# OzAmram/CaloDiffusion

Measured on AMD Instinct MI355X. Metric: sampled showers/sec (Dataset-2, 400-step DDIM), higher is better.
Workload: dtype f32 (convs: fp32 operands as 2-term fp16 splits on the fp16 MFMA pipe, fp32 accumulate; attention/norms fp32)

## Files before the change

### calodiffusion_amd/build.py

```python
from __future__ import annotations

import os
import subprocess
import sys
from concurrent.futures import ThreadPoolExecutor

HERE = os.path.dirname(os.path.abspath(__file__))
CSRC = os.path.join(HERE, "csrc")
LIBDIR = os.path.join(HERE, "lib")
TAG = os.environ.get("CD_BUILD_TAG", "")
LIB = os.path.join(LIBDIR, f"libcalodiff_hip{'_' + TAG if TAG else ''}.so")
SOURCES = ["kernels_conv.hip", "kernels_conv_zs.hip", "kernels_attn.hip", "kernels_conv_small.hip", "kernels_deep.hip", "kernels_wgrad16.hip", "kernels_norm_attn.hip", "kernels_misc.hip", "kernels_mlp.hip", "kernels_mlp_train.hip", "kernels_bwd.hip", "profiler.hip", "plan.hip",
           "forward.hip", "sampler.hip", "train.hip", "bns.hip", "ops.hip", "misc_abi.hip"]
HIPCC = os.environ.get("HIPCC", "/opt/rocm/bin/hipcc")
FLAGS = ["--offload-arch=gfx950", "-O3", "-std=c++17", "-fPIC", "-fno-gpu-rdc", "-Wall", "-Wno-unused-function", "-Wno-unused-value"]
FLAGS += os.environ.get("CD_EXTRA_HIPCC_FLAGS", "").split()
FILE_FLAGS = {"kernels_conv_zs.hip": ["-mllvm", "-amdgpu-mfma-vgpr-form"]}


def _file_digest(paths, extra: str = "") -> str:
    import hashlib
    h = hashlib.sha256(extra.encode())
    for f in paths:
        h.update(os.path.basename(f).encode())
        h.update(open(f, "rb").read())
    return h.hexdigest()


def _read(path: str):
    try:
        return open(path).read().strip()
    except OSError:
        return None


def build_all(force: bool = False, verbose: bool = True) -> str:
    os.makedirs(LIBDIR, exist_ok=True)
    objdir = os.path.join(LIBDIR, "obj" + ("_" + TAG if TAG else ""))
    os.makedirs(objdir, exist_ok=True)
    inc = os.path.join(os.path.dirname(HERE), "include")
    headers = sorted(os.path.join(CSRC, f) for f in os.listdir(CSRC) if f.endswith((".h", ".inc")))
    headers += sorted(os.path.join(inc, f) for f in os.listdir(inc) if f.endswith(".h"))
    jobs = []
    objs = []
    for src in SOURCES:
        sp = os.path.join(CSRC, src)
        op = os.path.join(objdir, src.replace(".hip", ".o"))
        objs.append(op)
        flags = [*FLAGS, *FILE_FLAGS.get(os.path.basename(sp), [])]
        key = _file_digest([sp] + headers, " ".join(flags))
        if force or not os.path.exists(op) or _read(op + ".hash") != key:
            jobs.append(([HIPCC, *flags, "-c", sp, "-o", op], op, key))

    def run(cmd):
        if verbose:
            print(" ".join(cmd), flush=True)
        r = subprocess.run(cmd, capture_output=True, text=True)
        if r.returncode != 0:
            raise RuntimeError(f"hipcc failed:\n{r.stdout}\n{r.stderr}")
        if verbose and r.stderr.strip():
            print(r.stderr, file=sys.stderr)

    def compile_one(job):
        cmd, op, key = job
        if os.path.exists(op + ".hash"):
            os.remove(op + ".hash")
        run(cmd)
        with open(op + ".hash", "w") as fh:
            fh.write(key + "\n")

    with ThreadPoolExecutor(max_workers=4) as ex:
        list(ex.map(compile_one, jobs))
    want = source_hash()
    if force or jobs or not os.path.exists(LIB) or _read(LIB + ".srchash") != want:
        if os.path.exists(LIB + ".srchash"):
            os.remove(LIB + ".srchash")
        run([HIPCC, "--offload-arch=gfx950", "-shared", "-fPIC", "-o", LIB, *objs])
        with open(LIB + ".srchash", "w") as fh:
            fh.write(want + "\n")
    return LIB


def source_hash() -> str:
    import hashlib
    h = hashlib.sha256((" ".join(FLAGS) + repr(sorted(FILE_FLAGS.items()))).encode())
    inc = os.path.join(os.path.dirname(HERE), "include")
    files = [os.path.join(CSRC, f) for f in sorted(os.listdir(CSRC))] + [os.path.join(inc, f) for f in sorted(os.listdir(inc))]
    for f in files:
        if f.endswith((".hip", ".h", ".inc")):
            h.update(os.path.basename(f).encode())
            h.update(open(f, "rb").read())
    return h.hexdigest()


if __name__ == "__main__":
    print(build_all(force="--force" in sys.argv))
```

### calodiffusion_amd/csrc/cd_common.h

```cpp
#pragma once
#include <hip/hip_runtime.h>
#include <stdint.h>
#include <stddef.h>
#include <string>

typedef float f32x4 __attribute__((ext_vector_type(4)));
typedef float f32x16 __attribute__((ext_vector_type(16)));

struct CdSamplerOp;

namespace cd {

void set_error(const std::string& msg);
struct Fail {
  int code;
  std::string msg;
};
#define CD_HIP(expr)                                                                                  \
  do {                                                                                                \
    hipError_t _e = (expr);                                                                           \
    if (_e != hipSuccess)                                                                             \
      throw cd::Fail{-2, std::string(#expr) + ": " + hipGetErrorString(_e)};                          \
  } while (0)
#define CD_REQUIRE(cond, msg)                                                                         \
  do {                                                                                                \
    if (!(cond)) throw cd::Fail{-1, std::string(msg)};                                                \
  } while (0)

namespace prof {
bool enabled();
void begin();
int end(char* buf, int cap);
struct Scope {
  Scope(const char* category, hipStream_t s, double flops, double bytes);
  ~Scope();
  int idx;
  hipStream_t stream;
};
}

enum ConvPrecision { PREC_F16X2 = 0, PREC_BF16X3 = 1, PREC_F32 = 2 };
int conv_precision();
void set_conv_precision(int p);
void set_conv_precision_override(int p);

struct Dims3 {
  int d, h, w;
  __host__ __device__ int64_t vox() const { return (int64_t)d * h * w; }
};

inline size_t packed_weight_floats(int cin, int cout, int taps) {
  return (size_t)(cin / 32) * taps * ((cout + 31) / 32) * 2048;
}

struct ConvGeom {
  Dims3 in, out;
  int kd, kh, kw;
  int sz, sh, sw;
};

__device__ __forceinline__ float cd_fast_silu(float t) {
  return t * __builtin_amdgcn_rcpf(1.f + __builtin_amdgcn_exp2f(t * -1.4426950408889634f));
}

struct GnDefer {
  const float* part = nullptr;
  int units = 0;
  const float* gamma = nullptr;
  const float* beta = nullptr;
  const float* add = nullptr;
  int add_ld = 0;
  int C = 0, groups = 0;
  int64_t vox = 0;
  float* coef_out = nullptr;
  float* stat_out = nullptr;
};

struct ConvFusion {
  const float* coef = nullptr;
  int act = 0;
  float* ch_part = nullptr;
  int* units = nullptr;
  const void* wpk_bf16x3 = nullptr;
  int* status = nullptr;
  GnDefer defer;
  float* coef_buf = nullptr;
  const unsigned* in_absmax = nullptr;
  const float* add_src = nullptr;
  int* add_done = nullptr;
  struct GnOut {
    const float* gamma = nullptr;
    const float* beta = nullptr;
    int groups = 0;
    const float* res0 = nullptr;
    const float* res1 = nullptr;
    int res_c0 = 0;
    float* part_out = nullptr;
    int* done = nullptr;
  } gn_out;
};
struct AbsmaxWords {
  unsigned* next = nullptr;
  unsigned* end = nullptr;
  unsigned* take() {
    CD_REQUIRE(next && next < end, "internal: out of max-|x| words");
    return next++;
  }
};
const unsigned* launch_absmax_bits(const float* x, size_t n, AbsmaxWords* words, hipStream_t s);
__host__ __device__ inline void pow2_scale_for(unsigned mb, float* scale, float* inv) {
  const int e = (int)((mb >> 23) & 0xff) - 127;
  int sexp = mb == 0u ? 0 : 10 - e;
  sexp = sexp < -100 ? -100 : (sexp > 100 ? 100 : sexp);
  union { unsigned u; float f; } a, b;
  a.u = (unsigned)(127 + sexp) << 23;
  b.u = (unsigned)(127 - sexp) << 23;
  *scale = a.f;
  *inv = b.f;
}
inline size_t packed_bf16x3_bytes(int cin, int cout, int taps) {
  return (size_t)(cin / 16) * taps * ((cout + 31) / 32) * 3 * 64 * 16;
}
inline size_t packed_f16x2_bytes(int cin, int cout, int taps) {
  return (size_t)(cin / 16) * taps * ((cout + 31) / 32) * 2 * 64 * 16;
}
inline size_t packed_split16_bytes(int cin, int cout, int taps) {
  return packed_bf16x3_bytes(cin, cout, taps) + packed_f16x2_bytes(cin, cout, taps);
}
void launch_pack_weights_bf16x3(const float* w_torch, void* wpk, int cout, int cin, int taps, hipStream_t s,
                                bool transposed = false, bool flip = false);
void launch_pack_weights_f16x2(const float* w_torch, void* wpk, int cout, int cin, int taps, hipStream_t s,
                               bool transposed = false, bool flip = false);
inline void launch_pack_weights_split16(const float* w_torch, void* wpk, int cout, int cin, int taps, hipStream_t s,
                                        bool transposed = false, bool flip = false) {
  launch_pack_weights_bf16x3(w_torch, wpk, cout, cin, taps, s, transposed, flip);
  launch_pack_weights_f16x2(w_torch, (char*)wpk + packed_bf16x3_bytes(cin, cout, taps), cout, cin, taps, s, transposed, flip);
}

void launch_pack_weights(const float* w_torch, float* wpk, int cout, int cin, int taps, bool transposed, hipStream_t s,
                         bool flip = false);
void launch_pack_init_weights(const float* w_torch, float* wpk, int cout, int cin, hipStream_t s);
struct PackJob {
  const float* src;
  float* raw;
  float* pk;
  void* bf3;
  void* f16;
  int cout, cin, taps;
  int kind;
  int tr, flip;
  unsigned long long numel, n_pk, n_bf3, n_f16;
};
void launch_pack_jobs(const PackJob* d_jobs, int njobs, hipStream_t s);
void launch_pack_jobs_f16x2(const PackJob* d_jobs, int njobs, hipStream_t s);

void launch_conv_mfma(const float* in0, int c0, const float* in1, int c1, const float* wpk, const float* bias, float* out,
                      int batch, int cout, const ConvGeom& g, hipStream_t s, const ConvFusion& fu = ConvFusion());
bool try_launch_conv_zslide(const float* in0, int c0, const float* in1, int c1, const void* wpk_f16x2, const float* bias, float* out,
                            int batch, int cout, const ConvGeom& g, hipStream_t s, const ConvFusion& fu);
bool try_launch_conv_small(const float* in0, int c0, const float* in1, int c1, const void* wpk_f16x2, const float* bias, float* out,
                           int batch, int cout, const ConvGeom& g, hipStream_t s, const ConvFusion& fu);
void launch_conv_transpose_mfma(const float* in, int cin, const float* wpk, const float* bias, float* out, int batch,
                                int cout, Dims3 din, Dims3 dout, int kz, int sz, hipStream_t s,
                                const void* wpk_f16x2 = nullptr, int* status = nullptr, const unsigned* in_absmax = nullptr);

enum A_Prologue { A_NONE = 0, A_AFFINE = 1, A_SOFTMAX32 = 2, A_EXPNORM = 3 };
struct PointwiseArgs {
  const float* in0 = nullptr;
  int ld0 = 0, off0 = 0, c0 = 0;
  const float* in1 = nullptr;
  int ld1 = 0, c1 = 0;
  const float* wpk = nullptr;
  int64_t w_batch_stride = 0;
  const float* bias = nullptr;
  const float* residual = nullptr;
  float* out = nullptr;
  int batch = 0, cout = 0;
  int64_t vox = 0;
  int prologue = A_NONE;
  const float* coef = nullptr;
  int out_ld = 0, out_off = 0;
  float* ch_part = nullptr;
  const float* gn_res = nullptr;
  GnDefer gn_defer;
  const void* wpk16 = nullptr;
  int* status = nullptr;
};
inline int pointwise_units(int64_t vox) { return (int)((vox + 127) / 128); }
void launch_pointwise(const PointwiseArgs& a, hipStream_t s);

struct InitConvArgs {
  const float* x = nullptr;
  int cx = 0;
  int cin = 0;
  const float* scale_b = nullptr;
  int scale_stride = 1;
  const float* sigma_b = nullptr;
  float sigma_data = 1.f;
  const float* r_w = nullptr;
  const float* z_d = nullptr;
  const float* phi_h = nullptr;
  int use_rz = 0, use_phi = 0;
  const float* wpk = nullptr;
  const float* bias = nullptr;
  float* out = nullptr;
  int batch = 0, cout = 0;
  Dims3 dims{};
  float* coord_table = nullptr;
  bool table_ready = false;
  int* status = nullptr;
};
void launch_init_conv(const InitConvArgs& a, hipStream_t s);
void launch_init_coord_table(const InitConvArgs& a, hipStream_t s);

int gn_nsplit_for(int64_t vox, int batch);
void launch_ch_stats(const float* x, float* part, int batch, int channels, int64_t vox, int nsplit, hipStream_t s);
void launch_gn_finalize(const float* part, int units, const float* gamma, const float* beta, const float* add_bc, int add_ld,
                        float* coef, int batch, int channels, int groups, int64_t vox, hipStream_t s,
                        float* stat_out = nullptr );

size_t wgrad_partial_floats(int64_t out_vox, int batch, bool per_sample, int A, int Bc, int T);
struct WgradReduceJob {
  const float* partial;
  float* dw;
  int A, Bc, T, nslots, flags , b_total, b_off;
  unsigned first_block;
};
struct WgradReduceQueue {
  static constexpr int kMax = 80;
  WgradReduceJob job[kMax];
  int n = 0;
  unsigned blocks = 0;
};
void wgrad_queue_flush(WgradReduceQueue* q, hipStream_t s);
struct WgradAux {
  WgradReduceQueue* queue = nullptr;
  AbsmaxWords* words = nullptr;
  const unsigned* gmax = nullptr;
  const unsigned* xmax = nullptr;
};
void launch_wgrad(const float* g, int A, Dims3 dg, const float* x, int Bc, int xld, int xoff, Dims3 dx, int kd, int kh, int kw,
                  int sz, int sxy, int batch, bool per_sample, float* partial, float* dw, bool accumulate, bool transposed_out,
                  hipStream_t s, int b_total = 0, int b_off = 0,
                  const float* xcoef = nullptr, const WgradAux& aux = WgradAux());
bool wgrad_x_norm_supported(Dims3 dg, Dims3 dx, int kd, int kh, int kw, int sz, int sxy);
bool wgrad_f16x2_eligible(Dims3 d);
bool try_launch_wgrad_f16x2(const float* g, int A, const float* x, int Bc, int xld, int xoff, Dims3 d, int batch, float* partial,
                            const WgradAux& aux, int* nblk_out, hipStream_t s, const float* xcoef = nullptr);
bool try_launch_wgrad_strided_f16x2(const float* g, int A, Dims3 dg, const float* x, int Bc, int xld, int xoff, Dims3 dx, int kd, int sz,
                                    int batch, float* partial, int max_slots, const WgradAux& aux, int* nblk_out, hipStream_t s);
void launch_strided_dgrad_naive(const float* dy, const float* w, float* dx, int batch, int cin, int cout, Dims3 din, Dims3 dout,
                                int kd, int sz, hipStream_t s);
void launch_softmax32(const float* qkv, float* qs, int64_t rows, hipStream_t s);
void launch_softmax32_bwd(const float* qs, const float* dqs, float* dqkv, int64_t rows, hipStream_t s);
void launch_ksoftmax_bwd(const float* qkv, const float* dks, const float* kstat, const float* ctx, const float* dctx, float dscale,
                         float* dqkv, int batch, int64_t vox, hipStream_t s);
void launch_pack_sample32(const float* m, float* wpk, int batch, bool transpose, float scale, hipStream_t s);
void launch_pack_sample32_pair(const float* m, float* wpk_plain, float* wpk_tr, int batch, float scale, hipStream_t s);
int head_bwd_blocks(int batch, int64_t vox);
void launch_head_loss_bwd(const float* x0, const float* data, const float* noise, const float* scal, const float* h, const float* wh,
                          float* dh, float* part, float* dwh, float* dbh, int batch, int64_t vox, hipStream_t s, int loss_type = 0,
                          int objective = 0);
void launch_head_vjp(const float* gy, const float* scal, const float* h, const float* wh, float* dh, float* part, float* dwh, float* dbh,
                     int batch, int64_t vox, int objective, hipStream_t s);
void launch_init_dgrad(const float* g, const float* w_raw, int cin, int c0, const float* gy, const float* scal, int objective, float* dx,
                       int batch, Dims3 dims, hipStream_t s);
struct LinearWgradJob {
  const float* delta;
  const float* in;
  float* dw;
  float* db;
  int nout, nin, delta_ld, in_ld;
};
void launch_linear_wgrad(const LinearWgradJob* jobs_dev, int njobs, int max_elems, int batch, hipStream_t s);
void launch_fold_phi(const float* src, float* dst, int batch, Dims3 d, int C, hipStream_t s);
void launch_add_slices(const float* a, int lda, int aoff, const float* b, int ldb, int boff, float* out, int channels,
                       int64_t rows, hipStream_t s);
void launch_bias_grad(const float* part, int units, int batch, int channels, float* db, bool accumulate, hipStream_t s);
size_t gn_backward_scratch_floats(int batch, int channels, int64_t vox);
struct GnParamJob {
  const float* sums_bc;
  float *dgamma, *dbeta, *dbias, *dsumdy;
  int batch, channels;
};
struct GnParamJobs {
  static constexpr int kMax = 64;
  GnParamJob job[kMax];
  int n = 0;
};
struct GnParamQueue {
  GnParamJobs jobs;
  float* sums = nullptr;
  float* sums_end = nullptr;
  float* next_sums = nullptr;
  bool discard = false;
};
void launch_gn_param_jobs(const GnParamJobs& jobs, hipStream_t s);
void launch_gn_backward(const float* dy, const float* h, const float* coef, const float* stat, const float* gamma, float* dh,
                        float* dgamma, float* dbeta, float* dadd, int dadd_ld, int batch, int channels, int64_t vox, int groups,
                        int silu, float* scratch, bool accumulate_params, hipStream_t s,
                        float* dbias = nullptr, float* dsumdy = nullptr,
                        GnParamQueue* queue = nullptr,
                        unsigned* dh_absmax = nullptr);
int gn_apply_blocks_per_sample(int batch, int channels, int64_t vox);
void launch_gn_apply(const float* x, float* y, const float* coef, int batch, int channels, int64_t vox, int silu,
                     const float* residual, const float* residual1, int res_c0, float* part_out, hipStream_t s,
                     const GnDefer* defer = nullptr);

int attn_nsplit_for(int64_t vox, int batch);
size_t attn_partial_floats(int batch, int nsplit);
void launch_attn_context(const float* qkv, float* partials, int batch, int64_t vox, int nsplit, hipStream_t s);
void launch_attn_combine(const float* partials, int nsplit, const float* w_out , int cout, float* wpk_b,
// ... 272 lines not shown
```

### calodiffusion_amd/csrc/kernels_conv.hip

```cpp
#include "cd_common.h"
#include "split16.h"
#include "gn_defer.h"
#include <cstdio>
#include <cstdlib>
#include <cstring>
#include <algorithm>
#include <map>
#include <string>
#include <vector>

namespace cd {

static int g_conv_precision = -1;
static thread_local int tl_conv_precision_override = -1;
void set_conv_precision_override(int p) { tl_conv_precision_override = p; }
int conv_precision() {
  if (tl_conv_precision_override >= 0) return tl_conv_precision_override;
  if (g_conv_precision < 0) {
    const char* e = getenv("CD_CONV_PRECISION");
    g_conv_precision = !e ? PREC_F16X2 : (!strcmp(e, "f32") ? PREC_F32 : (!strcmp(e, "bf16x3") ? PREC_BF16X3 : PREC_F16X2));
  }
  return g_conv_precision;
}
void set_conv_precision(int p) { g_conv_precision = p; }
// ... 1476 lines not shown
  const bool bf16x3 = prec != 0;
  if (getenv("CD_NO_FLAT")) return false;
  int geo = -1;
  if (g.kd == 3 && g.kh == 3 && g.kw == 3 && g.sz == 1 && g.sh == 1 && g.sw == 1) geo = 0;
  else if (g.kd == 3 && g.kh == 4 && g.kw == 4 && g.sh == 2 && g.sw == 2 && (g.sz == 1 || g.sz == 2)) geo = g.sz == 2 ? 1 : 2;
  else if (g.kd == 4 && g.kh == 4 && g.kw == 4 && g.sh == 2 && g.sw == 2 && g.sz == 2) geo = 3;
  if (geo < 0 || (geo != 0 && !bf16x3)) return false;
  const Dims3 d = g.in;
  const int CTtot = cout / 32;
  const int CTmax = CTtot <= 3 ? CTtot : 2;
  if (CTtot % CTmax) return false;
  const int HW = d.h * d.w, HWo = g.out.h * g.out.w;
  const size_t vox_bytes = prec == 3 ? 96 : (prec == 2 ? 80 : 64);
  auto planes = [&](int NT) { return ((32 * NT - 1) / HWo + 1) * g.sz + g.kd; };
  auto launch = [&](int NT, int VT, int CT) -> bool {
    if (VT < 0) {
      const int NLW = -VT;
      ConvFlatArgs a;
      a.in0 = in0; a.in1 = in1; a.c0 = c0; a.c1 = c1; a.wpk = (const float*)wpk; a.bias = bias; a.out = out;
      a.D = d.d; a.H = d.h; a.W = d.w; a.Do = g.out.d; a.Ho = g.out.h; a.Wo = g.out.w;
      a.R = 32 * NT; a.P = planes(NT); a.cout = cout; a.CTtot = CTtot; a.dbg = 0;
      a.coef = fu.coef; a.act = fu.act; a.ch_part = fu.ch_part;
      const size_t lds = 2 * ((size_t)a.P * HW + 1) * 96 + (size_t)NT * CT * 64 * 4;
      const int ups = (int)((g.out.vox() + a.R - 1) / a.R);
      const int total = ups * batch;
      const int nblk = total < 256 ? total : 256;
      dim3 grid((unsigned)nblk, 1, (unsigned)(CTtot / CT));
      if (fu.units) *fu.units = ups;
      const int threads = (NT + NLW) * 64;
      switch (CT) {
        case 1: launch_ws_inst<1>(a, grid, threads, lds, NLW, ups, total, s, geo); break;
        case 2: launch_ws_inst<2>(a, grid, threads, lds, NLW, ups, total, s, geo); break;
        case 3: launch_ws_inst<3>(a, grid, threads, lds, NLW, ups, total, s, geo); break;
        default: return false;
      }
      return true;
    }
    ConvFlatArgs a;
    a.in0 = in0; a.in1 = in1; a.c0 = c0; a.c1 = c1; a.wpk = (const float*)wpk; a.bias = bias; a.out = out;
    a.D = d.d; a.H = d.h; a.W = d.w; a.Do = g.out.d; a.Ho = g.out.h; a.Wo = g.out.w;
    a.R = 32 * NT; a.P = planes(NT); a.cout = cout; a.CTtot = CTtot;
    a.dbg = getenv("CD_FLAT_DBG") ? atoi(getenv("CD_FLAT_DBG")) : 0;
    a.coef = fu.coef; a.act = fu.act; a.ch_part = fu.ch_part; a.status = fu.status; a.in_absmax = fu.in_absmax;
    a.add_src = prec >= 2 && !bias ? fu.add_src : nullptr;
    size_t lds = ((size_t)a.P * HW + 1) * vox_bytes;
    const size_t red = (size_t)(NT / VT) * CT * 32 * 2 * 4;
    if (lds < red) lds = red;
    if (fu.defer.part) {
      lds = (lds + 15) & ~(size_t)15;
      a.defer = fu.defer;
      a.coef_lds_off = (int)lds;
      lds += (size_t)fu.defer.C * 16 + gn_defer_scratch_bytes(fu.defer.C);
      if (lds > 160 * 1024) return false;
    }
    dim3 grid((unsigned)((g.out.vox() + a.R - 1) / a.R), (unsigned)batch, (unsigned)(CTtot / CT));
    if (fu.units) *fu.units = (int)grid.x;
    const int threads = (NT / VT) * 64;
#define CD_FLAT_CASE(V, C)                                                   \
  if (VT == V && CT == C) {                                                  \
    if (prec == 3) launch_flat3_inst<V, C, 3>(a, grid, threads, lds, s, geo); \
    else if (prec == 2) {                                                    \
      if constexpr (V * C <= 4) launch_flat3_inst<V, C, 2>(a, grid, threads, lds, s, geo); \
      else return false;                                                     \
    } else launch_flat_inst<V, C>(a, grid, threads, lds, s);                 \
    if (a.add_src && fu.add_done) *fu.add_done = 1;                          \
    return true;                                                             \
  }
    CD_FLAT_CASE(1, 1) CD_FLAT_CASE(2, 1) CD_FLAT_CASE(3, 1) CD_FLAT_CASE(4, 1)
    CD_FLAT_CASE(1, 2) CD_FLAT_CASE(2, 2) CD_FLAT_CASE(3, 2) CD_FLAT_CASE(4, 2)
    CD_FLAT_CASE(1, 3) CD_FLAT_CASE(2, 3)
#undef CD_FLAT_CASE
    return false;
  };
  if (const char* ov = getenv("CD_FLAT_TILE")) {
    int nt, vt;
    if (sscanf(ov, "%d,%d", &nt, &vt) == 2 && nt % vt == 0 && nt / vt <= 8 && vt * CTmax <= 8 &&
        ((size_t)planes(nt) * HW + 1) * vox_bytes <= 160 * 1024 && (prec != 2 || vt * CTmax <= 4))
      return launch(nt, vt, CTmax);
  }
  static const int kCand[][2] = {{8, 2}, {4, 1}, {8, 1}, {12, 3}, {16, 2}, {16, 4}, {4, 2}, {6, 2}, {6, 3}, {2, 1},
                                 {3, 1}, {1, 1}, {2, 2}, {12, 2}, {8, 4}, {6, 1}, {3, 3}};
  struct Cand { int nt, vt, ct; };
  std::vector<Cand> cand;
  const bool small = g.out.vox() * batch <= 64 * 1024;
  for (int pass = 0; pass < (small && CTmax > 1 ? 2 : 1); ++pass) {
    const int CT = pass == 0 ? CTmax : 1;
    for (auto& c : kCand) {
      const int NT = c[0], VT = c[1];
      if (VT * CT > 8 || (CT == 3 && VT > 2)) continue;
      if (prec == 2 && VT * CT > 4) continue;
      static const bool no_extra_waves = getenv("CD_FLAT_NO_EXTRA_WAVES") != nullptr;
      const bool extra_ok = !no_extra_waves && g.out.vox() <= 128 && VT == 1 && NT <= 8;
      if ((int64_t)32 * (NT - 1) >= g.out.vox() && !extra_ok) continue;
      if (((size_t)planes(NT) * HW + 1) * vox_bytes > 150 * 1024) continue;
      if (pass == 1 && NT > 4) continue;
      cand.push_back({NT, VT, CT});
    }
  }
  if (prec == 3 && !getenv("CD_NO_WS")) {
    static const int kWs[][2] = {{8, 4}, {8, 2}, {4, 2}, {4, 4}, {8, 3}, {6, 2}, {2, 2}, {3, 1}, {1, 1}, {2, 1}};
    for (auto& c : kWs) {
      const int NMW = c[0], NLW = c[1];
      if ((int64_t)32 * (NMW - 1) >= g.out.vox()) continue;
      const size_t lds = 2 * ((size_t)planes(NMW) * HW + 1) * 96 + (size_t)NMW * CTmax * 64 * 4;
      if (lds > 160 * 1024 - 256) continue;
      cand.push_back({NMW, -NLW, CTmax});
    }
  }
  if (cand.empty()) return false;
  char key[192];
  std::snprintf(key, sizeof key, "flat%s g%d %dx%dx%d c%d+%d->%d b%d", prec == 3 ? "_bf16x3" : (prec == 2 ? "_f16x2" : "_f32"), geo,
                d.d, d.h, d.w, c0, c1, cout, batch);
  const int pick = autotune(key, (int)cand.size(), [&](int i) { launch(cand[i].nt, cand[i].vt, cand[i].ct); }, s);
  const Cand& c = cand[pick < 0 ? 0 : pick];
  return launch(c.nt, c.vt, c.ct);
}

void launch_conv_mfma(const float* in0, int c0, const float* in1, int c1, const float* wpk, const float* bias, float* out,
                      int batch, int cout, const ConvGeom& g, hipStream_t s, const ConvFusion& fu_in) {
  CD_REQUIRE((!fu_in.coef && !fu_in.defer.part) || c1 == 0, "conv: a fused input normalisation needs a single (non-concatenated) source");
  if (fu_in.units) *fu_in.units = 0;
  CD_REQUIRE(c0 % 32 == 0 && c1 % 32 == 0 && c0 > 0, "conv: channel counts must be multiples of 32");
  CD_REQUIRE(cout % 32 == 0, "conv: output channels must be a multiple of 32");
  CD_REQUIRE(g.kw <= 4, "conv: r kernel extent > 4 unsupported");
  const int CTtot = cout / 32;
  int CT = CTtot <= 3 ? CTtot : 2;
  CD_REQUIRE(CTtot % CT == 0, "conv: unsupported output channel count");
  char cat[128];
  std::snprintf(cat, sizeof cat, "conv%dx%dx%d_s%d C%d->%d @%dx%dx%d", g.kd, g.kh, g.kw, g.sh, c0 + c1, cout, g.in.d, g.in.h, g.in.w);
  const double taps = (double)g.kd * g.kh * g.kw;
  prof::Scope scope(cat, s, 2.0 * taps * (c0 + c1) * cout * (double)g.out.vox() * batch,
                    4.0 * batch * ((double)g.in.vox() * (c0 + c1) + (double)g.out.vox() * cout));
  ConvFusion fu = fu_in;
  auto materialise = [&]() {
    if (!fu.defer.part) return;
    if (fu.defer.coef_out) fu.coef_buf = fu.defer.coef_out;
    CD_REQUIRE(fu.coef_buf, "conv: deferred normalisation needs a coefficient buffer for kernels without the prologue");
    launch_gn_finalize(fu.defer.part, fu.defer.units, fu.defer.gamma, fu.defer.beta, fu.defer.add, fu.defer.add_ld, fu.coef_buf, batch,
                       fu.defer.C, fu.defer.groups, fu.defer.vox, s, fu.defer.stat_out);
    fu.coef = fu.coef_buf;
    fu.defer = GnDefer();
  };
  {
    const bool want_f32 = conv_precision() == PREC_F32, want_bf16x3 = conv_precision() == PREC_BF16X3;
    if (fu.wpk_bf16x3 && !want_f32 && !want_bf16x3 &&
        try_launch_conv_zslide(in0, c0, in1, c1, (const char*)fu.wpk_bf16x3 + packed_bf16x3_bytes(c0 + c1, cout, g.kd * g.kh * g.kw),
                               bias, out, batch, cout, g, s, fu))
      return;
    if (fu.wpk_bf16x3 && !want_f32 && !want_bf16x3 &&
        try_launch_conv_small(in0, c0, in1, c1, (const char*)fu.wpk_bf16x3 + packed_bf16x3_bytes(c0 + c1, cout, g.kd * g.kh * g.kw),
                              bias, out, batch, cout, g, s, fu))
      return;
    if (fu.wpk_bf16x3 && !want_f32 && !want_bf16x3 &&
        try_launch_conv3_flat(in0, c0, in1, c1, (const char*)fu.wpk_bf16x3 + packed_bf16x3_bytes(c0 + c1, cout, g.kd * g.kh * g.kw), bias,
                              out, batch, cout, g, s, fu, 2))
      return;
    materialise();
    if (fu.wpk_bf16x3 && !want_f32 && try_launch_conv3_flat(in0, c0, in1, c1, fu.wpk_bf16x3, bias, out, batch, cout, g, s, fu, 3))
      return;
    if (try_launch_conv3_flat(in0, c0, in1, c1, wpk, bias, out, batch, cout, g, s, fu, 0)) return;
  }
  {
    const bool want_f32 = conv_precision() == PREC_F32;
    if (fu.wpk_bf16x3 && !want_f32) {
      const bool f16_ok = conv_precision() == PREC_F16X2 && !fu.in_absmax;
      for (int pass = f16_ok ? 0 : 1; pass < 2; ++pass) {
      const bool f16 = pass == 0;
      const std::vector<ConvTile> cand3 = conv_tile_candidates(g, batch, CT, 14, f16 ? 80 : 96);
      auto launch3 = [&](const ConvTile& t) {
        ConvTiled3Args a3;
        ConvKArgs& a = a3.k;
        a3.status = fu.status;
        a.in0 = in0; a.in1 = in1; a.c0 = c0; a.c1 = c1; a.bias = bias; a.out = out;
        a.wpk = f16 ? (const float*)((const char*)fu.wpk_bf16x3 + packed_bf16x3_bytes(c0 + c1, cout, g.kd * g.kh * g.kw))
                    : (const float*)fu.wpk_bf16x3;
        a.Din = g.in.d; a.Hin = g.in.h; a.Win = g.in.w; a.Do = g.out.d; a.Ho = g.out.h; a.Wo = g.out.w;
        a.KD = g.kd; a.KH = g.kh; a.KW = g.kw; a.SZ = g.sz; a.SH = g.sh; a.SW = g.sw;
        a.TZ = t.TZ; a.TH = t.TH; a.nTZ = (g.out.d + t.TZ - 1) / t.TZ; a.nTH = (g.out.h + t.TH - 1) / t.TH;
        a.IZ = (t.TZ - 1) * g.sz + g.kd; a.IH = (t.TH - 1) * g.sh + g.kh;
        a.cout = cout; a.CTtot = CTtot; a.coef = fu.coef; a.act = fu.act;
        const int units = a.nTZ * a.nTH;
        const int64_t cap = (g.out.vox() + 31) / 32;
        a3.ch_part = (fu.ch_part && units <= cap) ? fu.ch_part : nullptr;
        if (fu.units) *fu.units = a3.ch_part ? units : 0;
        dim3 grid((unsigned)(batch * a.nTZ * a.nTH), (unsigned)(CTtot / CT));
        size_t lds = t.lds;
        const size_t red = (size_t)t.NW * CT * 32 * 2 * 4;
        if (lds < red) lds = red;
        if (f16) {
          if (t.VT == 1 && CT == 1) { launch_tiled3_inst<1, 1, 2>(a3, grid, t.NW * 64, lds, s); return; }
          if (t.VT == 2 && CT == 1) { launch_tiled3_inst<2, 1, 2>(a3, grid, t.NW * 64, lds, s); return; }
          if (t.VT == 1 && CT == 2) { launch_tiled3_inst<1, 2, 2>(a3, grid, t.NW * 64, lds, s); return; }
          CD_REQUIRE(false, "conv: no f16x2 tiled kernel instance for the chosen tiling");
        }
#define CD_T3_CASE(V, C)                                              \
  if (t.VT == V && CT == C) {                                         \
    launch_tiled3_inst<V, C>(a3, grid, t.NW * 64, lds, s);            \
    return;                                                           \
  }
        CD_T3_CASE(1, 1) CD_T3_CASE(2, 1) CD_T3_CASE(3, 1) CD_T3_CASE(4, 1)
        CD_T3_CASE(1, 2) CD_T3_CASE(2, 2) CD_T3_CASE(3, 2) CD_T3_CASE(4, 2)
        CD_T3_CASE(1, 3) CD_T3_CASE(2, 3)
#undef CD_T3_CASE
        CD_REQUIRE(false, "conv: no bf16x3 tiled kernel instance for the chosen tiling");
      };
      std::vector<ConvTile> ok;
      for (auto& t : cand3)
        if (f16 ? (t.VT * CT <= 2) : (t.VT <= 4 && !(CT == 3 && t.VT > 2))) ok.push_back(t);
      if (!ok.empty()) {
        char key3[192];
        std::snprintf(key3, sizeof key3, "tiled_%s %s b%d", f16 ? "f16x2" : "bf16x3", cat, batch);
        const int pick3 = autotune(key3, (int)ok.size(), [&](int i) { launch3(ok[i]); }, s);
        launch3(ok[pick3 < 0 ? 0 : pick3]);
        return;
      }
      }
    }
  }
  const std::vector<ConvTile> cand = conv_tile_candidates(g, batch, CT, 14);
  auto launch = [&](const ConvTile& t) {
    ConvKArgs a;
    a.in0 = in0; a.in1 = in1; a.c0 = c0; a.c1 = c1; a.wpk = wpk; a.bias = bias; a.out = out;
    a.Din = g.in.d; a.Hin = g.in.h; a.Win = g.in.w; a.Do = g.out.d; a.Ho = g.out.h; a.Wo = g.out.w;
    a.KD = g.kd; a.KH = g.kh; a.KW = g.kw; a.SZ = g.sz; a.SH = g.sh; a.SW = g.sw;
    a.TZ = t.TZ; a.TH = t.TH; a.nTZ = (g.out.d + t.TZ - 1) / t.TZ; a.nTH = (g.out.h + t.TH - 1) / t.TH;
    a.IZ = (t.TZ - 1) * g.sz + g.kd; a.IH = (t.TH - 1) * g.sh + g.kh;
    a.cout = cout; a.CTtot = CTtot; a.coef = fu.coef; a.act = fu.act;
    dim3 grid((unsigned)(batch * a.nTZ * a.nTH), (unsigned)(CTtot / CT));
    const int threads = t.NW * 64;
#define CD_CONV_CASE(V, C)                                        \
  if (t.VT == V && CT == C) {                                     \
    launch_conv_inst<V, C>(a, grid, threads, t.lds, s);           \
    return;                                                       \
  }
    CD_CONV_CASE(1, 1) CD_CONV_CASE(2, 1) CD_CONV_CASE(3, 1) CD_CONV_CASE(4, 1)
    CD_CONV_CASE(5, 1) CD_CONV_CASE(6, 1) CD_CONV_CASE(7, 1) CD_CONV_CASE(8, 1)
    CD_CONV_CASE(1, 2) CD_CONV_CASE(2, 2) CD_CONV_CASE(3, 2) CD_CONV_CASE(4, 2)
    CD_CONV_CASE(1, 3) CD_CONV_CASE(2, 3)
#undef CD_CONV_CASE
    CD_REQUIRE(false, "conv: no kernel instance for the chosen tiling");
  };
  char key[192];
  std::snprintf(key, sizeof key, "tiled %s b%d", cat, batch);
  int pick = autotune(key, (int)cand.size(), [&](int i) { launch(cand[i]); }, s);
  launch(cand[pick < 0 ? 0 : pick]);
  return;
#define CD_CONV_CASE(V, C)
#undef CD_CONV_CASE
  CD_REQUIRE(false, "conv: no kernel instance for the chosen tiling");
}

struct ConvTArgs {
  const float* in;
  int cin;
  const float* wpk;
  const float* bias;
  float* out;
  int Din, Hin, Win, Do, Ho, Wo;
  int KZ, SZ;
  int cout, CTtot;
  int TZ, TH, nTZ, nTH;
  int Cw;
  int CS;
  const u32x4* wpk16;
  int* status;
  const unsigned* in_absmax;
  int tr_off = 0;
};

template <int CT>
__global__ void __launch_bounds__(256) conv_transpose_kernel(ConvTArgs a) {
  extern __shared__ __attribute__((aligned(16))) float lds[];
  const int tid = threadIdx.x, lane = tid & 63, wave = tid >> 6, nw = blockDim.x >> 6;
  int bid = blockIdx.x;
  const int thi = bid % a.nTH;
  bid /= a.nTH;
  const int tzi = bid % a.nTZ;
  const int b = bid / a.nTZ;
  const int a0 = tzi * a.TZ, b0 = thi * a.TH;
  const int PZ = a.TZ + 2, PH = a.TH + 2;
  const int tileVox = PZ * PH * a.Win;
  const int ZERO = tileVox * a.CS;
  const int half = lane >> 5, col = lane & 31;
  for (int i = tid; i < a.CS; i += blockDim.x) lds[ZERO + i] = 0.f;

  {
    const int c4 = a.cin >> 2;
    const int items = tileVox * c4;
    const float* src = a.in + (size_t)b * a.Din * a.Hin * a.Win * a.cin;
    for (int idx = tid; idx < items; idx += blockDim.x) {
      const int q = idx % c4, vox = idx / c4;
      const int iw = vox % a.Win;
      const int r = vox / a.Win;
      const int lh = r % PH, lz = r / PH;
      const int gz = a0 - 1 + lz;
      int gh = (b0 - 1 + lh) % a.Hin;
      if (gh < 0) gh += a.Hin;
      f32x4 val = {0.f, 0.f, 0.f, 0.f};
      if (gz >= 0 && gz < a.Din) val = *(const f32x4*)(src + ((size_t)(gz * a.Hin + gh) * a.Win + iw) * a.cin + q * 4);
      *(f32x4*)(lds + vox * a.CS + q * 4) = val;
    }
  }
  __syncthreads();

  const int ncls = a.SZ * 4;
  const int njt = (a.TZ * a.TH * a.Cw + 31) / 32;
// ... 806 lines not shown
```

### calodiffusion_amd/engine.py

```python
from __future__ import annotations

import ctypes as C
import os
from typing import Dict, Optional, Sequence

import numpy as np
import torch

_HERE = os.path.dirname(os.path.abspath(__file__))
LIB_PATH = os.environ.get("CALODIFF_LIB") or os.path.join(_HERE, "lib", "libcalodiff_hip.so")

CD_MAX_SIZES = 8
CD_ABI_VERSION = 3
TIME_KINDS = {"log": 0, "sigma": 1, "raw": 2}
OBJECTIVES = {"hybrid": 0, "noise_pred": 1, "mean_pred": 2}
LOSS_TYPES = {"l2": 0, "l1": 1, "mse": 2, "huber": 3}


class CdUnetDesc(C.Structure):
    _fields_ = [
        ("struct_size", C.c_uint32),
        ("grid", C.c_int32 * 3),
        ("in_channels", C.c_int32),
        ("n_sizes", C.c_int32),
# ... 116 lines not shown
    _check_built_from_these_sources()
    lib = C.CDLL(LIB_PATH)
    for name, (res, args) in _SIGNATURES.items():
        fn = getattr(lib, name)
        fn.restype, fn.argtypes = res, args
    if lib.cd_abi_version() != CD_ABI_VERSION:
        raise RuntimeError(f"{LIB_PATH} reports ABI version {lib.cd_abi_version()}, this binding is written against "
                           f"{CD_ABI_VERSION} (include/calodiff.h): rebuild with `python -m calodiffusion_amd.build`")
    _lib = lib
    return lib


def _check_built_from_these_sources():
    if os.environ.get("CALODIFF_LIB") or os.environ.get("CD_SKIP_SRCHASH"):
        return
    from . import build
    stamp = LIB_PATH + ".srchash"
    have = open(stamp).read().strip() if os.path.exists(stamp) else None
    want = build.source_hash()
    if have != want:
        raise RuntimeError(f"{LIB_PATH} was not built from the sources in {build.CSRC} (stamp {str(have)[:12]}, sources "
                           f"{want[:12]}): run `python -m calodiffusion_amd.build`")


def _check(code: int):
    if code != 0:
        msg = load_library().cd_last_error().decode(errors="replace")
        exc = ValueError if code == -1 else RuntimeError
        raise exc(f"calodiff[{code}]: {msg}")


def require_gpu() -> str:
    lib = load_library()
    if not torch.cuda.is_available():
        raise RuntimeError("calodiffusion_amd needs an MI355X (gfx950) GPU: torch.cuda.is_available() is False and "
                           "there is no CPU fallback")
    buf = C.create_string_buffer(256)
    _check(lib.cd_device_check(buf, 256))
    return buf.value.decode()


def _ptr(t: Optional[torch.Tensor]) -> Optional[int]:
    return None if t is None else t.data_ptr()


def _stream() -> int:
    return torch.cuda.current_stream().cuda_stream


def _dev32(t: torch.Tensor, name: str) -> torch.Tensor:
    if not isinstance(t, torch.Tensor) or not t.is_cuda:
        raise RuntimeError(f"{name} must be a CUDA(ROCm) tensor: calodiffusion_amd computes on the GPU only")
    if t.dtype != torch.float32 or not t.is_contiguous():
        t = t.to(torch.float32).contiguous()
    return t


def _i32x3(v: Sequence[int]):
    return (C.c_int32 * 3)(*[int(a) for a in v])


class UnetEngine:

    def __init__(self, unet, rz_input=False, phi_input=False, time_kind="raw", objective="hybrid", sigma_data=1.0,
                 coords=None):
        self.lib = load_library()
        self.device_name = require_gpu()
        self.unet = unet
        d = CdUnetDesc()
        d.struct_size = C.sizeof(CdUnetDesc)
        d.grid = _i32x3(unet.grid)
        d.in_channels = unet.channels
        d.n_sizes = len(unet.layer_sizes)
        for i, v in enumerate(unet.layer_sizes):
            d.layer_sizes[i] = int(v)
        d.groups = unet.groups
        d.block_attn = int(bool(unet.block_attn))
        d.mid_attn = int(unet.mid_attn is not False)
        d.compress_z = int(bool(unet.compress_Z))
        d.cond_size, d.cond_dim = unet.cond_size, unet.cond_dim
        d.rz_input, d.phi_input = int(bool(rz_input)), int(bool(phi_input))
        d.time_embed_kind = TIME_KINDS[time_kind]
        d.objective = OBJECTIVES[objective]
        d.sigma_data = float(sigma_data)
        d.time_sin, d.cond_sin = int(bool(getattr(unet, "time_embed", False))), int(bool(getattr(unet, "cond_embed", False)))
        self.desc = d
        self.grid = tuple(unet.grid)
        self.voxels = int(np.prod(self.grid))
        handle = _P()
        _check(self.lib.cd_plan_create(C.byref(d), C.byref(handle)))
        self.plan = handle
        self._weights_version = None
        self._weight_order = None
        self._weight_ids = None
        self._held_weights = []
        self._ws: Dict[tuple, torch.Tensor] = {}
        self.device = next(unet.parameters()).device
        if self.device.type != "cuda":
            raise RuntimeError("move the model to the GPU first (model.to('cuda')): calodiffusion_amd has no CPU path")
        if coords is not None:
            r, z, phi = (np.ascontiguousarray(a, dtype=np.float32) for a in coords)
            assert len(r) == self.grid[2] and len(z) == self.grid[0] and len(phi) == self.grid[1]
            _check(self.lib.cd_plan_set_coords(self.plan, r.ctypes.data, z.ctypes.data, phi.ctypes.data, _stream()))
        self.sync_weights(force=True)

    @classmethod
    def for_unet(cls, unet):
        opts = getattr(unet, "_engine_opts", {})
        return cls(unet, **opts)

    def __del__(self):
        try:
            if getattr(self, "plan", None):
                self.lib.cd_plan_destroy(self.plan)
                self.plan = None
        except Exception:
            pass

    def _version(self):
        ps = list(self.unet.parameters())
        return tuple(p._version for p in ps) + tuple(p.data_ptr() for p in ps) + (tuple(id(p) for p in ps),)

    def sync_weights(self, force=False):
        ver = self._version()
        if not force and ver == self._weights_version:
            return
        ids = ver[-1]
        if self._weight_order is None or self._weight_ids != ids:
            sd = self.unet.state_dict(keep_vars=True)
            n = C.c_int()
            _check(self.lib.cd_plan_num_weights(self.plan, C.byref(n)))
            buf = C.create_string_buffer(256)
            numel = C.c_int64()
            order = []
            for i in range(n.value):
                _check(self.lib.cd_plan_weight_name(self.plan, i, buf, 256, C.byref(numel)))
                name = buf.value.decode()
                if name not in sd:
                    raise RuntimeError(f"state_dict has no tensor named {name!r}")
                if sd[name].numel() != numel.value:
                    raise RuntimeError(f"{name}: {sd[name].numel()} elements, HIP plan expects {numel.value}")
                order.append((name, sd[name]))
            missing = set(sd) - {name for name, _ in order}
            if missing:
                raise RuntimeError(f"HIP plan does not consume these state_dict tensors: {sorted(missing)[:5]} ...")
            self._weight_order, self._weight_ids = order, ids
        tensors = [_dev32(t.detach(), name) for name, t in self._weight_order]
        ptrs = (_P * len(tensors))(*[t.data_ptr() for t in tensors])
        _check(self.lib.cd_plan_set_weights(self.plan, len(tensors), ptrs, _stream()))
        self._held_weights = tensors
        self._weights_version = ver

    _WS_SWITCHES = ("CD_NO_DEEP_LEVEL", "CD_NO_PW_CLOSE", "CD_NO_FUSED_ATTN", "CD_NO_GNDEFER", "CD_ATTN_COMBINE_LAUNCH", "CD_PW_F32",
                    "CD_NO_ATTN_MOMENTS", "CD_ATTN_MOM_MIN")

    def _ws_key(self, batch: int):
        return (int(batch),) + tuple(os.environ.get(k) for k in self._WS_SWITCHES)

    def workspace(self, batch: int) -> torch.Tensor:
        key = ("net",) + self._ws_key(batch)
        ws = self._ws.get(key)
        if ws is None:
            nbytes = C.c_size_t()
            _check(self.lib.cd_plan_workspace_bytes(self.plan, batch, C.byref(nbytes)))
            self._ws = {k: v for k, v in self._ws.items() if k[0] != "net"}
            ws = torch.empty(nbytes.value, dtype=torch.uint8, device=self.device)
            self._ws[key] = ws
        return ws

    def unet_forward(self, x, cond, time):
        x, cond, time = _dev32(x, "x"), _dev32(cond, "cond"), _dev32(time, "time")
        B = x.shape[0]
        if tuple(x.shape[1:]) != (self.unet.channels,) + self.grid:
            raise ValueError(f"x has shape {tuple(x.shape)}, expected (B, {self.unet.channels}, {self.grid})")
        if self.desc.cond_sin:
            if cond.numel() != B:
                raise ValueError("cond_embed='sin' takes cond of shape (B,)")
        elif cond.shape != (B, self.unet.cond_size):
            raise ValueError("cond must be (B, cond_size)")
        if time.numel() != B:
            raise ValueError("time must be (B,)")
        self.sync_weights()
        ws = self.workspace(B)
        out = torch.empty((B, 1) + self.grid, dtype=torch.float32, device=x.device)
        _check(self.lib.cd_unet_forward(self.plan, B, x.data_ptr(), cond.data_ptr(), time.data_ptr(), out.data_ptr(),
                                        ws.data_ptr(), ws.numel(), _stream()))
        return out

    safe_denoise = True

    def denoise(self, x, sigma, cond):
        x, cond = _dev32(x, "x"), _dev32(cond, "cond")
        B = x.shape[0]
        sigma = _dev32(sigma, "sigma").reshape(-1)
        if sigma.numel() == 1 and B > 1:
            sigma = sigma.expand(B).contiguous()
        if tuple(x.shape[1:]) != (1,) + self.grid or sigma.numel() != B or cond.shape != (B, self.unet.cond_size):
            raise ValueError(f"denoise shapes: x {tuple(x.shape)}, sigma {tuple(sigma.shape)}, cond {tuple(cond.shape)}")
        self.sync_weights()
        ws = self.workspace(B)
        out = torch.empty_like(x)
        if self.safe_denoise:
            fell = C.c_int(0)
            _check(self.lib.cd_denoise_safe(self.plan, B, x.data_ptr(), sigma.data_ptr(), cond.data_ptr(), out.data_ptr(),
                                            ws.data_ptr(), ws.numel(), C.byref(fell), _stream()))
            if fell.value:
                self.range_fallbacks = getattr(self, "range_fallbacks", 0) + 1
        else:
            _check(self.lib.cd_denoise(self.plan, B, x.data_ptr(), sigma.data_ptr(), cond.data_ptr(), out.data_ptr(),
                                       ws.data_ptr(), ws.numel(), _stream()))
        return out

    def ddim_sample(self, start, cond, steps: np.ndarray, step_noise=None, seed=0, offset=0, debug=False, use_graph=True,
                    out=None, noise_stride=0):
        start, cond = _dev32(start, "start"), _dev32(cond, "cond")
        B = start.shape[0]
        steps = np.ascontiguousarray(steps, dtype=np.float32)
        n_steps = steps.shape[0]
        assert steps.shape == (n_steps, 4)
        self.sync_weights()
        ws = self.workspace(B)
        x_out = torch.empty_like(start) if out is None else out
        xs = x0s = None
        if debug:
            xs = torch.empty((n_steps,) + tuple(start.shape), dtype=torch.float32, device=start.device)
            x0s = torch.empty_like(xs)
        if step_noise is not None:
            step_noise = _dev32(step_noise, "step_noise")
            assert step_noise.shape[0] == n_steps and step_noise[0].numel() == start.numel()
        _check(self.lib.cd_ddim_sample(self.plan, B, start.data_ptr(), cond.data_ptr(),
                                       steps.ctypes.data_as(C.POINTER(CdStep)), n_steps, _ptr(step_noise), int(seed),
                                       int(offset), int(noise_stride), x_out.data_ptr(), _ptr(xs), _ptr(x0s),
                                       int(bool(use_graph)), ws.data_ptr(), ws.numel(), _stream()))
        self.check_status()
        return x_out, xs, x0s

    def sampler_run(self, start, cond, program, step_noise=None, seed=0, offset=0, noise_stride=0, debug=False, use_graph=True):
        start, cond = _dev32(start, "start"), _dev32(cond, "cond")
        B = start.shape[0]
        coefs = np.ascontiguousarray(program.coefs, dtype=np.float32)
        n_steps, n_coef = coefs.shape
        ops = (CdSamplerOp * len(program.ops))()
        for o, (kind, dst, src, col) in zip(ops, program.ops):
            o.kind, o.dst, o.nsrc, o.col = kind, dst, len(src), col
            for j, v in enumerate(src):
                o.src[j] = v
        op_begin = None
        if program.op_begin is not None:
            assert len(program.op_begin) == n_steps + 1
            op_begin = (C.c_int32 * (n_steps + 1))(*program.op_begin)
        self.sync_weights()
        nbytes = C.c_size_t()
        _check(self.lib.cd_plan_sampler_workspace_bytes(self.plan, B, program.n_bufs, n_steps, n_coef, C.byref(nbytes)))
        key = ("sampler",) + self._ws_key(B)
        ws = self._ws.get(key)
        if ws is None or ws.numel() < nbytes.value:
            self._ws = {k: v for k, v in self._ws.items() if k[0] != "sampler"}
            ws = torch.empty(nbytes.value, dtype=torch.uint8, device=self.device)
            self._ws[key] = ws
        x_out = torch.empty_like(start)
        xs = x0s = None
        if debug:
            kinds = [(k, d) for k, d, _, _ in program.ops if k == SOP_RECORD]
            if (SOP_RECORD, 0) in kinds:
                xs = torch.zeros((n_steps,) + tuple(start.shape), dtype=torch.float32, device=start.device)
            if (SOP_RECORD, 1) in kinds:
                x0s = torch.zeros((n_steps,) + tuple(start.shape), dtype=torch.float32, device=start.device)
        if step_noise is not None:
            step_noise = _dev32(step_noise, "step_noise")
            assert step_noise.numel() == program.n_randn * start.numel(), "step_noise: one (B,1,D,H,W) tensor per RANDN op executed"
        _check(self.lib.cd_sampler_run(self.plan, B, start.data_ptr(), float(program.start_scale), cond.data_ptr(), program.n_bufs,
                                       n_steps, ops, len(program.ops), op_begin, coefs.ctypes.data, n_coef, _ptr(step_noise),
                                       int(seed), int(offset), int(noise_stride), x_out.data_ptr(), _ptr(xs), _ptr(x0s),
                                       int(bool(use_graph)), ws.data_ptr(), ws.numel(), _stream()))
        self.check_status()
        return x_out, xs, x0s

    def check_status(self):
        flags = C.c_int(0)
        _check(self.lib.cd_plan_status(self.plan, C.byref(flags), _stream()))
        if flags.value & 2:
            self.range_fallbacks = getattr(self, "range_fallbacks", 0) + 1
        if flags.value & 1:
            raise FloatingPointError("calodiff: an activation exceeded the fp16 range of the f16x2 convolution kernels "
                                     "(outputs contain inf/NaN); set CD_CONV_PRECISION=bf16x3 for the full fp32 range")

    def grad_layout(self):
        if getattr(self, "_grad_layout", None) is None:
            n = C.c_int()
            _check(self.lib.cd_plan_num_weights(self.plan, C.byref(n)))
            buf = C.create_string_buffer(256)
            numel, off, total = C.c_int64(), C.c_int64(), C.c_int64()
            lay = {}
            for i in range(n.value):
                _check(self.lib.cd_plan_weight_name(self.plan, i, buf, 256, C.byref(numel)))
                _check(self.lib.cd_plan_grad_layout(self.plan, i, C.byref(off), C.byref(total)))
                lay[buf.value.decode()] = (off.value, numel.value)
            self._grad_layout = (lay, total.value)
        return self._grad_layout

    def train_workspace(self, batch: int) -> torch.Tensor:
        ws = getattr(self, "_tws", {}).get(batch)
        if ws is None:
            nbytes = C.c_size_t()
            _check(self.lib.cd_plan_train_workspace_bytes(self.plan, batch, C.byref(nbytes)))
            ws = torch.empty(nbytes.value, dtype=torch.uint8, device=self.device)
            self._tws = {batch: ws}
# ... 421 lines not shown
```

Measured before the change: 92.88.

## Add plane-streaming 3x3x3 conv kernel for 32-voxel planes with LDS z-ring

Adds a specialised f16x2-split MFMA convolution for 3x3x3 stride-1 convs whose H*W plane is 32 voxels and whose input has 32 or 64 channels. Each block streams along z, keeps a four-slot LDS ring of split input planes and holds the weights in registers. Waves are split over channel slices and kz taps, and partial sums are reduced through LDS. GroupNorm/SiLU prologue, bias and channel-moment partials are fused in. It is tried ahead of the existing flat conv path to cut redundant input loads and launch overhead for the small first-level convs. The cost is many syncthreads per plane and low parallelism, since the grid is only chunks x batch x cout/32.

```diff
diff --git a/calodiffusion_amd/build.py b/calodiffusion_amd/build.py
--- a/calodiffusion_amd/build.py
+++ b/calodiffusion_amd/build.py
@@ -10,7 +10,7 @@
 LIBDIR = os.path.join(HERE, "lib")
 TAG = os.environ.get("CD_BUILD_TAG", "")
 LIB = os.path.join(LIBDIR, f"libcalodiff_hip{'_' + TAG if TAG else ''}.so")
-SOURCES = ["kernels_conv.hip", "kernels_conv_zs.hip", "kernels_attn.hip", "kernels_conv_small.hip", "kernels_deep.hip", "kernels_wgrad16.hip", "kernels_norm_attn.hip", "kernels_misc.hip", "kernels_mlp.hip", "kernels_mlp_train.hip", "kernels_bwd.hip", "profiler.hip", "plan.hip",
+SOURCES = ["kernels_conv.hip", "kernels_conv_zs.hip", "kernels_conv_l1.hip", "kernels_attn.hip", "kernels_conv_small.hip", "kernels_deep.hip", "kernels_wgrad16.hip", "kernels_norm_attn.hip", "kernels_misc.hip", "kernels_mlp.hip", "kernels_mlp_train.hip", "kernels_bwd.hip", "profiler.hip", "plan.hip",
            "forward.hip", "sampler.hip", "train.hip", "bns.hip", "ops.hip", "misc_abi.hip"]
 HIPCC = os.environ.get("HIPCC", "/opt/rocm/bin/hipcc")
 FLAGS = ["--offload-arch=gfx950", "-O3", "-std=c++17", "-fPIC", "-fno-gpu-rdc", "-Wall", "-Wno-unused-function", "-Wno-unused-value"]
diff --git a/calodiffusion_amd/csrc/cd_common.h b/calodiffusion_amd/csrc/cd_common.h
--- a/calodiffusion_amd/csrc/cd_common.h
+++ b/calodiffusion_amd/csrc/cd_common.h
@@ -158,6 +158,8 @@
                       int batch, int cout, const ConvGeom& g, hipStream_t s, const ConvFusion& fu = ConvFusion());
 bool try_launch_conv_zslide(const float* in0, int c0, const float* in1, int c1, const void* wpk_f16x2, const float* bias, float* out,
                             int batch, int cout, const ConvGeom& g, hipStream_t s, const ConvFusion& fu);
+bool try_launch_conv_plane32(const float* in0, int c0, const float* in1, int c1, const void* wpk_f16x2, const float* bias, float* out,
+                             int batch, int cout, const ConvGeom& g, hipStream_t s, const ConvFusion& fu);
 bool try_launch_conv_small(const float* in0, int c0, const float* in1, int c1, const void* wpk_f16x2, const float* bias, float* out,
                            int batch, int cout, const ConvGeom& g, hipStream_t s, const ConvFusion& fu);
 void launch_conv_transpose_mfma(const float* in, int cin, const float* wpk, const float* bias, float* out, int batch,
diff --git a/calodiffusion_amd/csrc/kernels_conv.hip b/calodiffusion_amd/csrc/kernels_conv.hip
--- a/calodiffusion_amd/csrc/kernels_conv.hip
+++ b/calodiffusion_amd/csrc/kernels_conv.hip
@@ -1652,6 +1652,10 @@
                               bias, out, batch, cout, g, s, fu))
       return;
     if (fu.wpk_bf16x3 && !want_f32 && !want_bf16x3 &&
+        try_launch_conv_plane32(in0, c0, in1, c1, (const char*)fu.wpk_bf16x3 + packed_bf16x3_bytes(c0 + c1, cout, g.kd * g.kh * g.kw),
+                                bias, out, batch, cout, g, s, fu))
+      return;
+    if (fu.wpk_bf16x3 && !want_f32 && !want_bf16x3 &&
         try_launch_conv3_flat(in0, c0, in1, c1, (const char*)fu.wpk_bf16x3 + packed_bf16x3_bytes(c0 + c1, cout, g.kd * g.kh * g.kw), bias,
                               out, batch, cout, g, s, fu, 2))
       return;
diff --git a/calodiffusion_amd/csrc/kernels_conv_l1.hip b/calodiffusion_amd/csrc/kernels_conv_l1.hip
--- /dev/null
+++ b/calodiffusion_amd/csrc/kernels_conv_l1.hip
@@ -0,0 +1,262 @@
+#include "cd_common.h"
+#include "split16.h"
+#include "gn_defer.h"
+
+#include <cstdio>
+#include <cstdlib>
+
+namespace cd {
+
+namespace {
+
+constexpr int P32_SLOTS = 4;
+constexpr int P32_ROW = 36;
+constexpr int P32_PART = 32 * P32_ROW * 4;
+
+struct ConvP32Args {
+  const float* in0;
+  const float* in1;
+  int c0, c1;
+  const u32x4* wpk;
+  int CTtot;
+  const float* bias;
+  float* out;
+  int cout;
+  const float* coef;
+  int act;
+  float* ch_part;
+  int* status;
+  GnDefer defer;
+  int D, H, W;
+  int nchunk;
+  int slot_bytes, ring_off, part_off, coef_off;
+};
+
+template <int KS>
+__global__ void __launch_bounds__(KS * 3 * 64) conv_plane32_f16x2_kernel(ConvP32Args a) {
+  extern __shared__ __attribute__((aligned(16))) float lds[];
+  char* ldsb = (char*)lds;
+  constexpr int CIN = KS * 16;
+  constexpr int NW = KS * 3;
+  constexpr int NT = NW * 64;
+  constexpr int VB = KS * 64 + 16;
+  constexpr int QPV = CIN / 4;
+  constexpr int NQ = 32 * QPV;
+  static_assert(NQ <= NT, "one staged quad per thread");
+  const int tid = threadIdx.x, lane = tid & 63;
+  const int wave = __builtin_amdgcn_readfirstlane(tid >> 6);
+  const int b = blockIdx.y, ct = blockIdx.z;
+  const int chunk = blockIdx.x;
+  const int D = a.D;
+  const int z0 = (int)(((long long)D * chunk) / a.nchunk), z1 = (int)(((long long)D * (chunk + 1)) / a.nchunk);
+  char* ring = ldsb + a.ring_off;
+  float* part = (float*)(ldsb + a.part_off);
+  float* ctab = (float*)(ldsb + a.coef_off);
+  const bool normed = a.coef || a.defer.part;
+
+  const int ks = wave / 3, kz = wave - ks * 3;
+  u32x4 w[9][2];
+#pragma unroll
+  for (int t = 0; t < 9; ++t)
+#pragma unroll
+    for (int te = 0; te < 2; ++te)
+      w[t][te] = a.wpk[((size_t)((ks * 27 + kz * 9 + t) * a.CTtot + ct) * 2 + te) * 64 + lane];
+
+  if (a.defer.part) {
+    gn_defer_to_lds(a.defer, b, ctab, ldsb + a.coef_off + CIN * 16);
+  } else if (a.coef) {
+    if (tid < CIN) *(f32x4*)(ctab + tid * 4) = *(const f32x4*)(a.coef + ((size_t)b * CIN + tid) * 4);
+  }
+  if (tid < P32_SLOTS * VB / 16) {
+    const int sl = tid / (VB / 16), k = tid - sl * (VB / 16);
+    *(f32x4*)(ring + sl * a.slot_bytes + 32 * VB + k * 16) = f32x4{0.f, 0.f, 0.f, 0.f};
+  }
+
+  const int half = lane >> 5, col = lane & 31;
+  int off9[9];
+  {
+    const int oh = col / a.W, ow = col - oh * a.W;
+#pragma unroll
+    for (int kh = 0; kh < 3; ++kh) {
+      int ih = oh + kh - 1;
+      ih = ih < 0 ? ih + a.H : (ih >= a.H ? ih - a.H : ih);
+#pragma unroll
+      for (int kw = 0; kw < 3; ++kw) {
+        const int iw = ow + kw - 1;
+        const int rec = (iw >= 0 && iw < a.W) ? ih * a.W + iw : 32;
+        off9[kh * 3 + kw] = rec * VB + half * 16 + ks * 64;
+      }
+    }
+  }
+
+  const int sv = (tid < NQ ? tid : tid - NQ) / QPV, sq = (tid < NQ ? tid : tid - NQ) - sv * QPV;
+  const int sch = sq * 4;
+  const float* src;
+  int ldc, coff;
+  if (sch < a.c0) {
+    src = a.in0; ldc = a.c0; coff = sch;
+  } else {
+    src = a.in1; ldc = a.c1; coff = sch - a.c0;
+  }
+  const size_t vox = (size_t)D * 32;
+  src += ((size_t)b * vox + sv) * ldc + coff;
+  const int sdst = sv * VB + (sch >> 4) * 64 + (sq & 3) * 8;
+  float amax = 0.f;
+  auto load_plane = [&](int zz) -> f32x4 {
+    const int zc = zz < 0 ? 0 : (zz >= D ? D - 1 : zz);
+    return *(const f32x4*)(src + (size_t)zc * 32 * ldc);
+  };
+  auto store_plane = [&](int zz, f32x4 v) {
+    if (tid >= NQ) return;
+    if (zz < 0 || zz >= D) v = f32x4{0.f, 0.f, 0.f, 0.f};
+    else if (normed) {
+      const f32x4* cf = (const f32x4*)(ctab + sch * 4);
+#pragma unroll
+      for (int e = 0; e < 4; ++e) {
+        const f32x4 c = cf[e];
+        float t = c[0] * v[e] + c[1];
+        if (a.act) t = cd_fast_silu(t);
+        v[e] = t + c[2];
+      }
+    }
+    amax = fmaxf(amax, fmaxf(fmaxf(fabsf(v[0]), fabsf(v[1])), fmaxf(fabsf(v[2]), fabsf(v[3]))));
+    u32x2 t1, t2;
+    split2(v, t1, t2);
+    char* d = ring + ((zz + P32_SLOTS) & (P32_SLOTS - 1)) * a.slot_bytes + sdst;
+    *(u32x2*)d = t1;
+    *(u32x2*)(d + 32) = t2;
+  };
+
+  {
+    f32x4 p0 = load_plane(z0 - 1), p1 = load_plane(z0), p2 = load_plane(z0 + 1);
+    __syncthreads();
+    store_plane(z0 - 1, p0);
+    store_plane(z0, p1);
+    store_plane(z0 + 1, p2);
+  }
+  __syncthreads();
+
+  const int ov = tid >> 3, oq = tid & 7;
+  f32x4 bias4 = f32x4{0.f, 0.f, 0.f, 0.f};
+  if (a.bias && tid < 256) bias4 = *(const f32x4*)(a.bias + ct * 32 + oq * 4);
+  f32x4 s1 = f32x4{0.f, 0.f, 0.f, 0.f}, s2 = s1;
+  float* outb = a.out + (size_t)b * vox * a.cout + ct * 32 + oq * 4;
+
+  for (int z = z0; z < z1; ++z) {
+    const f32x4 nxt = load_plane(z + 2);
+    __builtin_amdgcn_sched_barrier(0);
+    const char* base = ring + ((z + kz - 1 + P32_SLOTS) & (P32_SLOTS - 1)) * a.slot_bytes;
+    f32x16 acc, accB;
+#pragma unroll
+    for (int r = 0; r < 16; ++r) acc[r] = accB[r] = 0.f;
+    u32x4 av[3][2];
+    auto load_a = [&](int t) {
+#pragma unroll
+      for (int te = 0; te < 2; ++te) av[t % 3][te] = *(const u32x4*)(base + off9[t] + te * 32);
+    };
+    load_a(0);
+    load_a(1);
+#pragma unroll
+    for (int t = 0; t < 9; ++t) {
+      if (t + 2 < 9) load_a(t + 2);
+      const int c = t % 3;
+      acc = MFMA_F16(av[c][0], w[t][0], acc);
+      accB = MFMA_F16(av[c][0], w[t][1], accB);
+      accB = MFMA_F16(av[c][1], w[t][0], accB);
+    }
+    float* pw = part + wave * (P32_PART / 4);
+#pragma unroll
+    for (int r = 0; r < 16; ++r) {
+      const int row = (r & 3) + 8 * (r >> 2) + 4 * half;
+      pw[row * P32_ROW + col] = acc[r] + accB[r] * (1.f / 2048.f);
+    }
+    store_plane(z + 2, nxt);
+    __syncthreads();
+    if (tid < 256) {
+      f32x4 o = *(const f32x4*)(part + ov * P32_ROW + oq * 4);
+#pragma unroll
+      for (int w2 = 1; w2 < NW; ++w2) o += *(const f32x4*)(part + w2 * (P32_PART / 4) + ov * P32_ROW + oq * 4);
+      o += bias4;
+      *(f32x4*)(outb + ((size_t)z * 32 + ov) * a.cout) = o;
+      s1 += o;
+      s2 += o * o;
+    }
+    __syncthreads();
+  }
+  if (a.status && amax > 65504.f) atomicOr(a.status, 1);
+
+  if (a.ch_part) {
+#pragma unroll
+    for (int m = 8; m < 64; m <<= 1)
+#pragma unroll
+      for (int e = 0; e < 4; ++e) {
+        s1[e] += __shfl_xor(s1[e], m, 64);
+        s2[e] += __shfl_xor(s2[e], m, 64);
+      }
+    if (tid < 256 && lane < 8) {
+      *(f32x4*)(part + (wave * 8 + lane) * 8) = s1;
+      *(f32x4*)(part + (wave * 8 + lane) * 8 + 4) = s2;
+    }
+    __syncthreads();
+    if (tid < 32) {
+      const int q = tid >> 2, e = tid & 3;
+      float t1 = 0.f, t2 = 0.f;
+#pragma unroll
+      for (int w2 = 0; w2 < 4; ++w2) {
+        t1 += part[(w2 * 8 + q) * 8 + e];
+        t2 += part[(w2 * 8 + q) * 8 + 4 + e];
+      }
+      float* dst = a.ch_part + (((size_t)b * a.nchunk + chunk) * a.cout + ct * 32 + tid) * 2;
+      dst[0] = t1;
+      dst[1] = t2;
+    }
+  }
+}
+
+template <int KS>
+void launch_p32_inst(const ConvP32Args& a, dim3 grid, size_t lds, hipStream_t s) {
+  static bool attr_set = false;
+  if (!attr_set) {
+    CD_HIP(hipFuncSetAttribute((const void*)conv_plane32_f16x2_kernel<KS>, hipFuncAttributeMaxDynamicSharedMemorySize, 160 * 1024));
+    attr_set = true;
+  }
+  hipLaunchKernelGGL((conv_plane32_f16x2_kernel<KS>), grid, dim3(KS * 3 * 64), lds, s, a);
+  CD_HIP(hipGetLastError());
+}
+
+}
+
+bool try_launch_conv_plane32(const float* in0, int c0, const float* in1, int c1, const void* wpk_f16x2, const float* bias, float* out,
+                             int batch, int cout, const ConvGeom& g, hipStream_t s, const ConvFusion& fu) {
+  if (getenv("CD_NO_PLANE32")) return false;
+  if (!(g.kd == 3 && g.kh == 3 && g.kw == 3 && g.sz == 1 && g.sh == 1 && g.sw == 1)) return false;
+  if (g.in.h * g.in.w != 32 || g.in.h < 2 || g.in.d < 1) return false;
+  const int cin = c0 + c1;
+  if ((cin != 32 && cin != 64) || cout % 32 || c0 % 16 || c1 % 16) return false;
+  if (fu.in_absmax || fu.add_src) return false;
+  if ((fu.coef || fu.defer.part) && c1 != 0) return false;
+  if (fu.defer.part && fu.defer.C != cin) return false;
+  const int KS = cin / 16;
+  const int CTtot = cout / 32;
+  int nchunk = (4 + CTtot - 1) / CTtot;
+  if (nchunk > g.in.d) nchunk = g.in.d;
+  const int VB = KS * 64 + 16;
+  ConvP32Args a;
+  a.slot_bytes = (33 * VB + 15) & ~15;
+  a.ring_off = 0;
+  a.part_off = P32_SLOTS * a.slot_bytes;
+  a.coef_off = a.part_off + 3 * KS * P32_PART;
+  const size_t lds = (size_t)a.coef_off + cin * 16 + gn_defer_scratch_bytes(cin);
+  if (lds > 160 * 1024) return false;
+  a.in0 = in0; a.in1 = in1; a.c0 = c0; a.c1 = c1;
+  a.wpk = (const u32x4*)wpk_f16x2; a.CTtot = CTtot; a.bias = bias; a.out = out; a.cout = cout;
+  a.coef = fu.coef; a.act = fu.act; a.ch_part = fu.ch_part; a.status = fu.status; a.defer = fu.defer;
+  a.D = g.in.d; a.H = g.in.h; a.W = g.in.w; a.nchunk = nchunk;
+  const dim3 grid((unsigned)nchunk, (unsigned)batch, (unsigned)CTtot);
+  if (KS == 2) launch_p32_inst<2>(a, grid, lds, s);
+  else launch_p32_inst<4>(a, grid, lds, s);
+  if (fu.units) *fu.units = fu.ch_part ? nchunk : 0;
+  return true;
+}
+
+}
diff --git a/calodiffusion_amd/engine.py b/calodiffusion_amd/engine.py
--- a/calodiffusion_amd/engine.py
+++ b/calodiffusion_amd/engine.py
@@ -292,7 +292,7 @@
         self._weights_version = ver
 
     _WS_SWITCHES = ("CD_NO_DEEP_LEVEL", "CD_NO_PW_CLOSE", "CD_NO_FUSED_ATTN", "CD_NO_GNDEFER", "CD_ATTN_COMBINE_LAUNCH", "CD_PW_F32",
-                    "CD_NO_ATTN_MOMENTS", "CD_ATTN_MOM_MIN")
+                    "CD_NO_ATTN_MOMENTS", "CD_ATTN_MOM_MIN", "CD_NO_PLANE32")
 
     def _ws_key(self, batch: int):
         return (int(batch),) + tuple(os.environ.get(k) for k in self._WS_SWITCHES)
```

New measurement: 93.61 (median of 6 runs). No clear change (+0.8%).
